# jeffreychou777/GenComm

Hardware: AMD Instinct MI355X
Metric: scenes/sec (higher is better)
Workload: dtype f32

## Files before the change

### gencomm_amd/csrc/gencomm_abi.hip

```cpp
#include "../../include/gencomm_hip.h"

#include "common.h"
#include "conv_kernels.h"
#include "detect_kernels.h"
#include "enhancer_host.h"
#include "fusion_kernels.h"
#include "msgext_host.h"
#include "noise_kernels.h"
#include "pillar_kernels.h"
#include "pfn_kernels.h"
#include "train_kernels.h"
#include "wgrad_h3_kernels.h"
#include "unet_bwd_host.h"
#include "unet_host.h"

#include <algorithm>
#include <atomic>
#include <map>
#include <mutex>
#include <string>
#include <stdlib.h>
#include <string.h>

namespace gc {
char* last_error_buf() {
  static thread_local char buf[512] = {0};
  return buf;
}
KernelTimer& kernel_timer() {
  static KernelTimer t;
  return t;
}
static std::atomic<long long> g_modes[MODE_COUNT] = {{0}, {0}, {0}, {2}, {-1}, {1}, {0}, {0}, {-1}, {1}, {16}};
static std::atomic<bool> g_klog_armed{false};
static std::mutex g_klog_mu;
static std::map<std::string, int> g_klog;
bool klog_armed() { return g_klog_armed.load(std::memory_order_relaxed); }
void klog_note(const char* name) {
  std::lock_guard<std::mutex> lk(g_klog_mu);
  ++g_klog[name];
}
Modes modes_snapshot() {
  Modes m;
  for (int i = 0; i < MODE_COUNT; ++i) m.v[i] = g_modes[i].load(std::memory_order_relaxed);
  return m;
}
}

using namespace gc;

extern "C" {

int gencomm_abi_version(void) { return GENCOMM_ABI_VERSION; }
#ifndef GENCOMM_BUILD_FLAGS
#define GENCOMM_BUILD_FLAGS "unknown"
#endif
const char* gencomm_build_info(void) { return GENCOMM_BUILD_FLAGS; }
const char* gencomm_last_error(void) { return last_error_buf(); }

int gencomm_set_mode(int key, long long value) {
  GC_CHECK_ARG(key >= 0 && key < MODE_COUNT, "unknown mode key");
  GC_CHECK_ARG(key != MODE_ARITH || (value >= 0 && value <= 3), "GENCOMM_MODE_ARITH: 0 (three-term f16-pipe path), 1 (exact fp32), 2 (bf16 denoise) or 3 (0 + two-term general convolutions)");
  GC_CHECK_ARG(key != MODE_SAMPLER || (value >= 0 && value <= 2), "GENCOMM_MODE_SAMPLER: 0 (automatic), 1 (direct) or 2 (latent)");
  GC_CHECK_ARG(key != MODE_TILE_WANT || value >= 0, "GENCOMM_MODE_TILE_WANT: 0 (automatic) or a positive workgroup count");
  GC_CHECK_ARG(key != MODE_TILE8 || value >= -1, "GENCOMM_MODE_TILE8: -1 (automatic), 0 (off) or a positive workgroup count");
  GC_CHECK_ARG(key != MODE_BWD_STREAMS || (value >= 0 && value <= 2), "GENCOMM_MODE_BWD_STREAMS: 0 (off), 1 (automatic) or 2 (always)");
  GC_CHECK_ARG(key != MODE_PERSIST || (value >= 0 && value <= 31), "GENCOMM_MODE_PERSIST: a mask of the five layer variants (0 .. 31)");
  g_modes[key].store(value, std::memory_order_relaxed);
  return GC_OK;
}
long long gencomm_get_mode(int key) {
  if (key < 0 || key >= MODE_COUNT) { fail(GC_ERR_ARG, "unknown mode key"); return -1; }
  return g_modes[key].load(std::memory_order_relaxed);
}

int gencomm_timer_num_kernels(void) { return KF_COUNT; }
const char* gencomm_timer_kernel_name(int family) { return kernel_family_name(family); }

int gencomm_timer_start_mask(unsigned long long mask, int capacity) {
  KernelTimer& t = kernel_timer();
  GC_CHECK_ARG(t.ev == nullptr, "timer already armed");
  GC_CHECK_ARG(mask != 0 && (mask >> KF_COUNT) == 0 && capacity >= 1 && capacity <= (1 << 20), "bad family mask / capacity");
  t.ev = new hipEvent_t[2 * (size_t)capacity];
  for (int i = 0; i < 2 * capacity; ++i) {
    if (hipEventCreate(&t.ev[i]) != hipSuccess) {
      for (int j = 0; j < i; ++j) (void)hipEventDestroy(t.ev[j]);
      delete[] t.ev;
      t.ev = nullptr;
      return fail(GC_ERR_HIP, "hipEventCreate failed");
    }
  }
  t.fam = new int[capacity];
  t.bytes = new double[capacity];
  t.mask = mask; t.cap = capacity; t.count = 0;
  return GC_OK;
}
int gencomm_timer_start(int family, int capacity) {
  GC_CHECK_ARG(family >= 0 && family < KF_COUNT, "bad family");
  return gencomm_timer_start_mask(1ull << family, capacity);
}

int gencomm_timer_stop_families(double* ms, int* launches, double* algorithmic_bytes, int n_families) {
  KernelTimer& t = kernel_timer();
  GC_CHECK_ARG(t.ev != nullptr, "timer not armed");
  GC_CHECK_ARG(n_families >= 0 && n_families <= KF_COUNT, "bad n_families");
  for (int f = 0; f < n_families; ++f) {
    if (ms) ms[f] = 0.0;
    if (launches) launches[f] = 0;
    if (algorithmic_bytes) algorithmic_bytes[f] = 0.0;
  }
  int rc = GC_OK;
  for (int i = 0; i < t.count; ++i) {
    float e = 0.f;
    if (hipEventSynchronize(t.ev[2 * i + 1]) != hipSuccess || hipEventElapsedTime(&e, t.ev[2 * i], t.ev[2 * i + 1]) != hipSuccess)
      rc = fail(GC_ERR_HIP, "event timing failed");
    const int f = t.fam[i];
    if (f < n_families) {
      if (ms) ms[f] += e;
      if (launches) launches[f] += 1;
      if (algorithmic_bytes) algorithmic_bytes[f] += t.bytes[i];
    }
  }
  for (int i = 0; i < 2 * t.cap; ++i) (void)hipEventDestroy(t.ev[i]);
  delete[] t.ev;
  delete[] t.fam;
  delete[] t.bytes;
  t = KernelTimer{};
  return rc;
}

int gencomm_timer_stop(double* total_ms, int* launches) {
  double ms[KF_COUNT];
  int n[KF_COUNT];
  const int rc = gencomm_timer_stop_families(ms, n, nullptr, KF_COUNT);
  double sum = 0.0;
  int cnt = 0;
  for (int f = 0; f < KF_COUNT; ++f) { sum += ms[f]; cnt += n[f]; }
  if (total_ms) *total_ms = sum;
  if (launches) *launches = cnt;
  return rc;
}

int gencomm_klog_start(void) {
  std::lock_guard<std::mutex> lk(g_klog_mu);
  g_klog.clear();
  g_klog_armed.store(true, std::memory_order_relaxed);
// ... 279 lines not shown
  prep_c16_kernel<<<cdiv(2 * 1152, 256), 256, 0, st>>>(w, scratch, transposed);
  Modes m = modes_snapshot();
  m.v[MODE_ARITH] = 1;
  const size_t plane = (size_t)H * W;
  for (int g = 0; g < 2; ++g) {
    Conv8Args a{};
    a.src[0] = x; a.src[1] = x + 8 * plane; a.src_ct = x_ct;
    a.w = scratch + g * 1152; a.bias = scratch + 2 * 1152;
    a.dst = y + (size_t)8 * g * plane; a.dst_ct = y_ct;
    a.H = a.Hin = H; a.W = a.Win = W;
    a.xcd = m.xcd();
    launch_conv8<2, false, false, 0>(m, pick_tile(m, n, H, W), a, n, st);
  }
  GC_HIP(hipGetLastError());
  return GC_OK;
}

static void launch_q_sample(const QSampleArgs& q, int n, bool philox, hipStream_t st) {
  TimedLaunch tl(KF_Q_SAMPLE, st);
  const dim3 qgrid((unsigned)std::max<long long>(1, std::min<long long>((q.per_agent / 64 + 255) / 256, 2048)), n);
  GC_KLOG(philox ? "q_sample_kernel<true> (in-kernel Philox)" : "q_sample_kernel<false> (explicit noise)");
  if (philox) q_sample_kernel<true><<<qgrid, 256, 0, st>>>(q);
  else q_sample_kernel<false><<<qgrid, 256, 0, st>>>(q);
}

int gencomm_q_sample_fwd(const float* sched_row, const float* feat, int n_feat_rows, const int* src_row,
                         const float* noise, unsigned long long seed, unsigned int stream_id,
                         float* out, int n, int C, int H, int W, void* stream) {
  GC_CHECK_ARG(sched_row && feat && src_row && out, "null pointer");
  GC_CHECK_ARG(n >= 1 && n <= 65535 && n_feat_rows >= 1 && C >= 1 && H >= 1 && W >= 1, "bad n/C/H/W");
  QSampleArgs q{feat, src_row, noise, sched_row, out, seed, stream_id, (long long)C * H * W, nullptr, nullptr};
  launch_q_sample(q, n, noise == nullptr, (hipStream_t)stream);
  GC_HIP(hipGetLastError());
  return GC_OK;
}

int gencomm_step_noise_fwd(const float* sched_row, unsigned long long seed, unsigned int stream_id, float* out,
                           int n, int C, int H, int W, int unrounded, void* stream) {
  GC_CHECK_ARG(sched_row && out, "null pointer");
  GC_CHECK_ARG(n >= 1 && n <= 65535 && C >= 2 && (C & 1) == 0 && H >= 1 && W >= 1, "bad n/C/H/W (C must be even)");
  StepNoiseArgs a{out, sched_row, seed, stream_id, C, H, W, unrounded ? 1 : 0, (long long)n * (C / 2) * H * ((W + 3) / 4)};
  const unsigned grid = (unsigned)std::max<long long>(1, std::min<long long>((a.items + 255) / 256, 65536));
  step_noise_kernel<<<grid, 256, 0, (hipStream_t)stream>>>(a);
  GC_HIP(hipGetLastError());
  return GC_OK;
}

int gencomm_denoise_fwd(const float* prepared, const float* sched,
                        const float* feat, int n_feat_rows, const int* src_row, const float* cond,
                        float* out, const float* noise0, const float* step_noise, unsigned long long seed,
                        int n, int C, int H, int W, int levels, int res_blocks, int attn_mask, int T,
                        void* workspace, long long workspace_bytes, void* stream) {
  return gencomm_denoise_fwd_dseed(prepared, sched, feat, n_feat_rows, src_row, cond, out, noise0, step_noise, seed, nullptr,
                                   n, C, H, W, levels, res_blocks, attn_mask, T, workspace, workspace_bytes, stream);
}

int gencomm_denoise_fwd_dseed(const float* prepared, const float* sched,
                              const float* feat, int n_feat_rows, const int* src_row, const float* cond,
                              float* out, const float* noise0, const float* step_noise, unsigned long long seed,
                              const unsigned long long* seed_dev,
                              int n, int C, int H, int W, int levels, int res_blocks, int attn_mask, int T,
                              void* workspace, long long workspace_bytes, void* stream) {
  UNetPlan p;
  if (const char* e = p.build(C, levels, res_blocks, attn_mask, T)) return fail(GC_ERR_ARG, e);
  if (int rc = check_dims(n, C, H, W)) return rc;
  GC_CHECK_ARG(prepared && sched && feat && src_row && cond && out && workspace, "null pointer");
  GC_CHECK_ARG(n_feat_rows >= 1, "n_feat_rows must be positive");
  GC_CHECK_ARG((noise0 == nullptr) == (step_noise == nullptr), "noise0 and step_noise must both be given or both be null");
  UNetWorkspace w;
  if (const char* e = w.build(p, n, H, W)) return fail(GC_ERR_ARG, e);
  if ((long long)w.total > workspace_bytes) return fail(GC_ERR_WORKSPACE, "workspace too small (see gencomm_denoise_workspace_bytes)");
  hipStream_t st = (hipStream_t)stream;
  const bool philox = noise0 == nullptr;
  const long long per_agent = (long long)C * H * W;

  UNetCall c{&p, &w, prepared, (char*)workspace, n, H, W, st, modes_snapshot()};
  if (int rc = check_bf16_mode(c.m, p, W)) return rc;
  GC_HIP(hipMemsetAsync(c.amax(), 0, 256, st));
  amax_kernel<<<256, 256, 0, st>>>(cond, (long long)n * 2 * H * W, c.amax());
  QSampleArgs q{feat, src_row, noise0, sched + (size_t)(T - 1) * 5, out, seed, (unsigned)T, per_agent, seed_dev, c.amax() + 1};
  launch_q_sample(q, n, philox, st);

  const long long smode = c.m.v[MODE_SAMPLER];
  const bool want_latent = smode == 2 || (smode == 0 && pick_tile(c.m, n, H, W) == TILE_64x16);
  const bool latent = want_latent && T >= 2 && (W % 4) == 0;
  if (!latent) {
    for (int i = 0; i < T; ++i) {
      const int t = T - 1 - i;
      ConvOutArgs co{};
      co.out = out;
      co.xt = out;
      co.sched = sched + (size_t)t * 5;
      co.noise = philox ? nullptr : step_noise + (size_t)i * n * per_agent;
      co.seed = seed;
      co.seed_dev = seed_dev;
      co.stream_id = (unsigned)t;
      const int post = t == 0 ? 0 : (philox ? 2 : 1);
      if (int rc = unet_enqueue(c, out, cond, t, post, co)) return rc;
    }
    return GC_OK;
  }
  const int nops = (int)p.ops.size();
  kmap_enqueue(c, cond);
  for (int i = 0; i < T; ++i) {
    const int t = T - 1 - i;
    ConvOutArgs co{};
    co.out = out;
    if (int rc = unet_enqueue_range(c, out, cond, t, 0, co, i == 0 ? 0 : 1, t == 0 ? nops : nops - 1, i != 0, i == 0)) return rc;
    if (t > 0) {
      const float* nz = philox ? nullptr : step_noise + (size_t)i * n * per_agent;
      if (int rc = latent_step_enqueue(c, sched + (size_t)t * 5, nz, seed, (unsigned)t, seed_dev)) return rc;
    }
  }
  return GC_OK;
}

int gencomm_enhancer_num_params(int C) {
  EnhancerPlan p;
  if (const char* e = p.build(C)) { fail(GC_ERR_ARG, e); return -1; }
  return (int)p.params.size();
}
int gencomm_enhancer_param_info(int C, int index, char* name, int name_cap, long long* numel, long long* offset) {
  EnhancerPlan p;
  if (const char* e = p.build(C)) return fail(GC_ERR_ARG, e);
  GC_CHECK_ARG(index >= 0 && index < (int)p.params.size(), "param index out of range");
  GC_CHECK_ARG(name && name_cap > 0 && numel && offset, "null output pointer");
  snprintf(name, (size_t)name_cap, "%s", p.params[index].name.c_str());
  *numel = p.params[index].numel;
  *offset = p.params[index].off;
  return GC_OK;
}
long long gencomm_enhancer_raw_floats(int C) {
  EnhancerPlan p;
  if (const char* e = p.build(C)) { fail(GC_ERR_ARG, e); return -1; }
  return p.raw_floats;
}
long long gencomm_enhancer_workspace_bytes(int n, int C, int H, int W) {
  EnhancerPlan p;
  if (const char* e = p.build(C)) { fail(GC_ERR_ARG, e); return -1; }
  if (n < 1 || H < 1 || W < 1) { fail(GC_ERR_ARG, "n, H, W must be positive"); return -1; }
  return (long long)enhancer_workspace_bytes(p, n, H, W);
}
int gencomm_enhancer_fwd(const float* raw, const float* x, float* out, int n, int C, int H, int W,
                         void* workspace, long long workspace_bytes, void* stream) {
  EnhancerPlan p;
  if (const char* e = p.build(C)) return fail(GC_ERR_ARG, e);
  GC_CHECK_ARG(raw && x && workspace, "null pointer");
  GC_CHECK_ARG(n >= 1 && n <= 65535 && H >= 1 && W >= 1, "bad n/H/W");
  if ((long long)enhancer_workspace_bytes(p, n, H, W) > workspace_bytes)
    return fail(GC_ERR_WORKSPACE, "workspace too small (see gencomm_enhancer_workspace_bytes)");
  return enhancer_enqueue(p, raw, x, out, n, H, W, (char*)workspace, (hipStream_t)stream, modes_snapshot());
}

int gencomm_msgext_num_params(int C) {
  MsgExtPlan p;
  if (const char* e = p.build(C)) { fail(GC_ERR_ARG, e); return -1; }
  return (int)p.params.size();
}
int gencomm_msgext_param_info(int C, int index, char* name, int name_cap, long long* numel, long long* offset) {
  MsgExtPlan p;
  if (const char* e = p.build(C)) return fail(GC_ERR_ARG, e);
  GC_CHECK_ARG(index >= 0 && index < (int)p.params.size(), "param index out of range");
  GC_CHECK_ARG(name && name_cap > 0 && numel && offset, "null output pointer");
  snprintf(name, (size_t)name_cap, "%s", p.params[index].name.c_str());
  *numel = p.params[index].numel;
  *offset = p.params[index].off;
  return GC_OK;
// ... 556 lines not shown
```

### gencomm_amd/csrc/latenth_kernels.h

```cpp
#pragma once
#include "conv8b_kernels.h"
#include "conv8h_kernels.h"
#include "latent_kernels.h"

namespace gc {

constexpr int HL_LH5 = HC_TH + 4;
constexpr int HL_PLANE5 = HL_LH5 * HC_ROW;
constexpr int HL_W5TAB3 = 8 * HC_WC3;
constexpr int HL_TPLANE5 = HL_PLANE5 / 2;
constexpr int HL_RING = (2 * (HC_TW + 4) + 2 * HL_LH5) * 8;

__global__ __launch_bounds__(256) void prep_latent_h_kernel(const float* __restrict__ wc5, const float* __restrict__ w_in ,
                                                           float* __restrict__ dst5, float* __restrict__ dstx,
                                                           float* __restrict__ dstc, int C) {
  __shared__ float s_max[256];
  const int tid = threadIdx.x;
  const int CI = C + 2;
  float m = 0.f;
  for (int i = tid; i < 1600; i += 256) m = fmaxf(m, fabsf(wc5[i]));
  for (int i = tid; i < 8 * CI * 9; i += 256) m = fmaxf(m, fabsf(w_in[i]));
  s_max[tid] = m;
  __syncthreads();
  for (int s = 128; s > 0; s >>= 1) {
// ... 337 lines not shown
    for (int i = 0; i < 4; ++i) b0[i] = (oc0 + i < C) ? a.bias[oc0 + i] * sc : 0.f;
#pragma unroll 1
    for (int rp = 0; rp < 2; ++rp) {
      f32x4 acc[2][4] = {{b0, b0, b0, b0}, {b0, b0, b0, b0}};
      const unsigned char* trow = tile + 2 * rp * HC_ROW;
#pragma unroll
      for (int c = 0; c < 3; ++c) {
        WA3 wa;
        load_wa3(wa, tab, c, lane);
        long bt[2][4];
#pragma unroll
        for (int r = 0; r < 2; ++r)
#pragma unroll
          for (int j = 0; j < 4; ++j) bt[r][j] = *reinterpret_cast<const long*>(tile + HC_TOFF + (((2 * rp + r) * HC_ROW + off[j][c]) >> 1));
#pragma unroll
        for (int r = 0; r < 2; ++r) {
          __builtin_amdgcn_sched_barrier(0);
#pragma unroll
          for (int j = 0; j < 4; ++j) acc[r][j] = __builtin_amdgcn_mfma_f32_16x16x32_bf8_bf8(wa.wb, bt[r][j], acc[r][j], 0, 0, 0);
        }
        __builtin_amdgcn_sched_barrier(0);
#pragma unroll
        for (int r = 0; r < 2; ++r) {
          half8_t bh[4], bl[4];
#pragma unroll
          for (int j = 0; j < 4; ++j) {
            bh[j] = *reinterpret_cast<const half8_t*>(trow + r * HC_ROW + off[j][c]);
            bl[j] = *reinterpret_cast<const half8_t*>(trow + r * HC_ROW + HC_PLANE + off[j][c]);
          }
#pragma unroll
          for (int j = 0; j < 4; ++j) acc[r][j] = __builtin_amdgcn_mfma_f32_16x16x32_f16(wa.w[2], bh[j], acc[r][j], 0, 0, 0);
#pragma unroll
          for (int j = 0; j < 4; ++j) acc[r][j] = __builtin_amdgcn_mfma_f32_16x16x32_f16(wa.w[1], bl[j], acc[r][j], 0, 0, 0);
#pragma unroll
          for (int j = 0; j < 4; ++j) acc[r][j] = __builtin_amdgcn_mfma_f32_16x16x32_f16(wa.w[1], bh[j], acc[r][j], 0, 0, 0);
#pragma unroll
          for (int j = 0; j < 4; ++j) acc[r][j] = __builtin_amdgcn_mfma_f32_16x16x32_f16(wa.w[0], bl[j], acc[r][j], 0, 0, 0);
#pragma unroll
          for (int j = 0; j < 4; ++j) acc[r][j] = __builtin_amdgcn_mfma_f32_16x16x32_f16(wa.w[0], bh[j], acc[r][j], 0, 0, 0);
          if (r == 0) __builtin_amdgcn_sched_barrier(0);
        }
      }
      __builtin_amdgcn_sched_barrier(0);
#pragma unroll
      for (int r = 0; r < 2; ++r) {
        const int gy = y0 + 4 * wave + 2 * rp + r;
        if (gy >= H || gx + 3 >= W) continue;
#pragma unroll
        for (int ip = 0; ip < 2; ++ip) {
          if (oc0 + 2 * ip >= C) continue;
          float z8[8];
          if (POST == 2)
            noise_pair_quad((uint64_t)(((size_t)n * C + oc0 + 2 * ip) * plane + (size_t)gy * W + gx), a.stream_id, seed, bm_k2(sg), z8);
#pragma unroll
          for (int ii = 0; ii < 2; ++ii) {
            const int i = 2 * ip + ii, oc = oc0 + i;
            const size_t e = ((size_t)n * C + oc) * plane + (size_t)gy * W + gx;
            float v[4];
#pragma unroll
            for (int j = 0; j < 4; ++j) v[j] = acc[r][j][i] * inv_s;
            if (POST != 0) {
              const float4 t4 = *reinterpret_cast<const float4*>(a.xt + e);
              const float xt[4] = {t4.x, t4.y, t4.z, t4.w};
              if (POST == 1) {
                const float4 z4 = *reinterpret_cast<const float4*>(a.noise + e);
                const float z[4] = {z4.x, z4.y, z4.z, z4.w};
#pragma unroll
                for (int j = 0; j < 4; ++j) v[j] = fmaf(sg, z[j], fmaf(c1, v[j], c2 * xt[j]));
              } else {
#pragma unroll
                for (int j = 0; j < 4; ++j) v[j] = z8[4 * ii + j] + fmaf(c1, v[j], c2 * xt[j]);
              }
            }
            *reinterpret_cast<float4*>(a.out + e) = make_float4(v[0], v[1], v[2], v[3]);
            if (POST != 0) amax = fmaxf(amax, fmaxf(fmaxf(fabsf(v[0]), fabsf(v[1])), fmaxf(fabsf(v[2]), fabsf(v[3]))));
          }
        }
      }
    }
  }
  if (POST != 0 && a.amax_out != nullptr) wave_amax_commit(amax, a.amax_out);
}

template <int NOISE>
__global__ __launch_bounds__(HC_NT, 3) void latent_step_h_kernel(const LatentArgs a) {
  constexpr int NT = HC_NT, TW = HC_TW, TH = HC_TH;
  constexpr int TILE_BYTES = NOISE == 1 ? 2 * HC_PLANE + HC_TPLANE : 2 * HL_PLANE5;
  __shared__ __align__(16) unsigned char tile[TILE_BYTES];
  __shared__ float s_ring[HL_RING];
  __shared__ float s_ab[8][2];
  __shared__ float s_red[NT / 64][16];

  fp16_ovfl_clamp();
  const int tid = threadIdx.x, lane = tid & 63, wave = tid >> 6;
  const BlockId bid = xcd_block(a.xcd);
  const int n = bid.z;
  const int x0 = bid.x * TW, y0 = bid.y * TH;
  const int H = a.H, W = a.W;
  const unsigned plane = (unsigned)(H * W);
  const float c1 = a.sched[2], c2 = a.sched[3], sg = a.sched[4];
  const unsigned long long seed = (NOISE == 2 && a.seed_dev) ? *a.seed_dev : a.seed;
  const int ln = lane & 15, g = lane >> 4, ch = g & 1, rr = g >> 1;
  const int gx = x0 + 4 * ln;
  const int gy0 = y0 + 4 * wave + rr;
  const bool wave_live = y0 + 4 * wave < H;

  const int af32 = !a.a_bf16;
  const size_t abase = (size_t)n * 8 * plane;
  float4 qm[8], qr[2];
  float hh[2][2];
  const int r0 = tid >> 4, qx = tid & 15;
  const bool ok_m = (y0 - 2 + r0) >= 0 && (y0 - 2 + r0) < H && (x0 + 4 * qx) < W;
#pragma unroll
  for (int c = 0; c < 8; ++c)
    qm[c] = ok_m ? ld4(a.a_src, af32, abase + ((unsigned)c * plane + (unsigned)(y0 - 2 + r0) * (unsigned)W + (unsigned)(x0 + 4 * qx)))
                 : make_float4(0.f, 0.f, 0.f, 0.f);
  const int rrow = TH + ((tid & 63) >> 4), cpr = tid >> 6;
  const bool ok_r = (y0 - 2 + rrow) >= 0 && (y0 - 2 + rrow) < H && (x0 + 4 * qx) < W;
#pragma unroll
  for (int k = 0; k < 2; ++k)
    qr[k] = ok_r ? ld4(a.a_src, af32, abase + ((unsigned)(2 * cpr + k) * plane + (unsigned)(y0 - 2 + rrow) * (unsigned)W + (unsigned)(x0 + 4 * qx)))
                 : make_float4(0.f, 0.f, 0.f, 0.f);
  bool ok_h[2];
#pragma unroll
  for (int j = 0; j < 2; ++j) {
    const int idx = tid + j * NT;
    const int cp = idx & 3, s = (idx >> 2) & 3, r = idx >> 4;
    const int gy = y0 - 2 + r, gxh = s < 2 ? x0 - 2 + s : x0 + TW + (s - 2);
    ok_h[j] = idx < HL_LH5 * 16 && gy >= 0 && gy < H && gxh >= 0 && gxh < W;
    hh[j][0] = hh[j][1] = 0.f;
    if (ok_h[j]) {
      hh[j][0] = ld1(a.a_src, af32, abase + (unsigned)(2 * cp) * plane + (unsigned)gy * (unsigned)W + (unsigned)gxh);
      hh[j][1] = ld1(a.a_src, af32, abase + (unsigned)(2 * cp + 1) * plane + (unsigned)gy * (unsigned)W + (unsigned)gxh);
    }
  }
  if (tid < 8) {
    float A, B;
    gn_coeff(a.a_stat + (size_t)n * 16, tid, 2, a.inv_cnt, a.gamma[tid], a.beta[tid], &A, &B);
    s_ab[tid][0] = A;
    s_ab[tid][1] = B;
  }
  __syncthreads();
  auto act = [&](int c, float v, bool ok) { return ok ? c1 * silu_f(fmaf(s_ab[c][0], v, s_ab[c][1])) : 0.f; };
  uint2 tq[4];
  uint32_t tr2[2];
  uint32_t th2;
  {
    float e[8][4];
#pragma unroll
    for (int c = 0; c < 8; ++c) {
      e[c][0] = act(c, qm[c].x, ok_m); e[c][1] = act(c, qm[c].y, ok_m); e[c][2] = act(c, qm[c].z, ok_m); e[c][3] = act(c, qm[c].w, ok_m);
    }
#pragma unroll
    for (int j = 0; j < 4; ++j) {
      uint4 hi, lo;
      float t[8];
      split3_pair(e[0][j], e[1][j], hi.x, lo.x, t[0], t[1]);
      split3_pair(e[2][j], e[3][j], hi.y, lo.y, t[2], t[3]);
      split3_pair(e[4][j], e[5][j], hi.z, lo.z, t[4], t[5]);
      split3_pair(e[6][j], e[7][j], hi.w, lo.w, t[6], t[7]);
      const int addr = r0 * HC_ROW + j * HC_PHASE + (qx + 1) * 16;
      *reinterpret_cast<uint4*>(tile + addr) = hi;
      *reinterpret_cast<uint4*>(tile + HL_PLANE5 + addr) = lo;
      tq[j] = make_uint2(bf8x4s(t[0], t[1], t[2], t[3]), bf8x4s(t[4], t[5], t[6], t[7]));
    }
  }
  {
// ... 67 lines not shown
  if (NOISE == 1) {
    stage_load<TW, TH, NT, 8, false>(R, np_, plane, W, H, W, x0, y0, tid);
    hreg = halo_load_h<false>(np_, plane, W, H, W, x0, y0, tid);
  }
  __syncthreads();

  const float inv_s = a.wc5h[HL_W5TAB3], sc = a.wc5h[HL_W5TAB3 + 1];
  f32x4 acc[2][4];
  {
    const float4 b4 = *reinterpret_cast<const float4*>(a.bsum + 4 * ch);
    const float k = c1 * sc;
    const f32x4 b0 = {b4.x * k, b4.y * k, b4.z * k, b4.w * k};
#pragma unroll
    for (int p = 0; p < 2; ++p)
#pragma unroll
      for (int j = 0; j < 4; ++j) acc[p][j] = b0;
  }
  auto addr5 = [&](int c, int p, int j) {
    const int t = min(4 * c + g, 29);
    const int dyp = t / 5, dx = t - 5 * dyp;
    const int po = j + dx - 2;
    return (4 * wave + dyp + 2 * p) * HC_ROW + (ln + 1) * 16 + (po & 3) * HC_PHASE + (po >> 2) * 16;
  };
  if (wave_live) {
#pragma unroll 2
    for (int c = 0; c < 8; ++c) {
      half8_t w[3];
#pragma unroll
      for (int k = 0; k < 3; ++k) w[k] = __builtin_bit_cast(half8_t, *reinterpret_cast<const uint4*>(a.wc5h + c * HC_WC3 + (k * 64 + lane) * 4));
#pragma unroll
      for (int p = 0; p < 2; ++p) {
        half8_t b[4];
#pragma unroll
        for (int j = 0; j < 4; ++j) b[j] = *reinterpret_cast<const half8_t*>(tile + addr5(c, p, j));
#pragma unroll
        for (int j = 0; j < 4; ++j) acc[p][j] = __builtin_amdgcn_mfma_f32_16x16x32_f16(w[2], b[j], acc[p][j], 0, 0, 0);
#pragma unroll
        for (int j = 0; j < 4; ++j) acc[p][j] = __builtin_amdgcn_mfma_f32_16x16x32_f16(w[1], b[j], acc[p][j], 0, 0, 0);
#pragma unroll
        for (int j = 0; j < 4; ++j) acc[p][j] = __builtin_amdgcn_mfma_f32_16x16x32_f16(w[0], b[j], acc[p][j], 0, 0, 0);
        __builtin_amdgcn_sched_barrier(0);
#pragma unroll
        for (int j = 0; j < 4; ++j) b[j] = *reinterpret_cast<const half8_t*>(tile + HL_PLANE5 + addr5(c, p, j));
#pragma unroll
        for (int j = 0; j < 4; ++j) acc[p][j] = __builtin_amdgcn_mfma_f32_16x16x32_f16(w[1], b[j], acc[p][j], 0, 0, 0);
#pragma unroll
        for (int j = 0; j < 4; ++j) acc[p][j] = __builtin_amdgcn_mfma_f32_16x16x32_f16(w[0], b[j], acc[p][j], 0, 0, 0);
        __builtin_amdgcn_sched_barrier(0);
      }
    }
  }

  if (wave_live) {
    hl_border_fix(a, s_ring, x0, y0, acc[0], gy0, gx, gy0 - y0, gx - x0, 4 * ch, c1, sc);
    hl_border_fix(a, s_ring, x0, y0, acc[1], gy0 + 2, gx, gy0 + 2 - y0, gx - x0, 4 * ch, c1, sc);
  }

  auto composite_third_term = [&](const unsigned char* tbase) {
    static_for<0, 8>([&](auto CC) {
      constexpr int c = decltype(CC)::value;
      const long wb = *reinterpret_cast<const long*>(a.wc5h + c * HC_WC3 + 768 + lane * 2);
      long bt[2][4];
#pragma unroll
      for (int p = 0; p < 2; ++p)
#pragma unroll
        for (int j = 0; j < 4; ++j) bt[p][j] = *reinterpret_cast<const long*>(tbase + (addr5(c, p, j) >> 1));
#pragma unroll
      for (int p = 0; p < 2; ++p) {
        __builtin_amdgcn_sched_barrier(0);
#pragma unroll
        for (int j = 0; j < 4; ++j) acc[p][j] = __builtin_amdgcn_mfma_f32_16x16x32_bf8_bf8(wb, bt[p][j], acc[p][j], 0, 0, 0);
      }
    });
    __builtin_amdgcn_sched_barrier(0);
  };
  __syncthreads();
  write_t_plane(tile + HL_PLANE5);
  __syncthreads();
  if (wave_live) composite_third_term(tile + HL_PLANE5);

  int off[4][3];
  hc_lane_offsets(off, wave, lane);
  const int nchunk = a.C / 8;
  if (NOISE == 2) {
    __syncthreads();
    write_t_plane(tile + HL_PLANE5);
  }
#pragma unroll 1
  for (int cc = 0; cc < nchunk; ++cc) {
    __syncthreads();
    const float* __restrict__ wtab = a.wxh + (size_t)cc * HC_WTAB3;
    if (NOISE == 1) {
      stage_store_h<false, true>(tile, R, hreg, H, W, x0, y0, nullptr, tid, sg);
      if (cc + 1 < nchunk) {
        stage_load<TW, TH, NT, 8, false>(R, np_ + (size_t)(cc + 1) * 8 * plane, plane, W, H, W, x0, y0, tid);
        hreg = halo_load_h<false>(np_ + (size_t)(cc + 1) * 8 * plane, plane, W, H, W, x0, y0, tid);
      }
    } else {
      const float k2 = bm_k2(sg);
      auto words = [&](int cp, int r, int gx2, NoiseWords& w) -> float {
        const int gy2 = y0 - 1 + r;
        noise_words((uint64_t)(((size_t)n * a.C + (size_t)cc * 8 + 2 * cp) * plane + (size_t)gy2 * W + gx2), a.stream_id, seed, w);
        return (gy2 >= 0 && gy2 < H && gx2 >= 0 && gx2 < W) ? k2 : 0.f;
      };
      {
        uint32_t h[4][4];
#pragma unroll
        for (int cp = 0; cp < 4; ++cp) {
          NoiseWords w;
          const float kk = words(cp, r0, x0 + 4 * qx, w);
#pragma unroll
          for (int j = 0; j < 4; ++j) h[cp][j] = bm_pair_h(w.ur[j], w.w[j], kk);
        }
#pragma unroll
        for (int j = 0; j < 4; ++j)
          *reinterpret_cast<uint4*>(tile + r0 * HC_ROW + j * HC_PHASE + (qx + 1) * 16) = make_uint4(h[0][j], h[1][j], h[2][j], h[3][j]);
      }
      {
        const int cr = tid >> 5, rrw = TH + ((tid >> 4) & 1);
        NoiseWords w;
        const float kk = words(cr >> 1, rrw, x0 + 4 * qx, w);
        const bool odd = (cr & 1) != 0;
        const int jb = odd ? 2 : 0;
        const uint32_t wsel[2] = {odd ? w.w[2] : w.w[0], odd ? w.w[3] : w.w[1]};
        const float usel[2] = {odd ? w.ur[2] : w.ur[0], odd ? w.ur[3] : w.ur[1]};
#pragma unroll
        for (int k = 0; k < 2; ++k)
          *reinterpret_cast<uint32_t*>(tile + rrw * HC_ROW + (jb + k) * HC_PHASE + (qx + 1) * 16 + (cr >> 1) * 4) = bm_pair_h(usel[k], wsel[k], kk);
      }
      if (tid < HC_LH * 8) {
        const int cp = tid & 3, side = (tid >> 2) & 1, r = tid >> 3;
        NoiseWords w;
        const float kk = words(cp, r, side ? x0 + TW : x0 - 4, w);
        *reinterpret_cast<uint32_t*>(tile + hc_addr(r, side ? HC_TW : -1) + cp * 4) = bm_pair_h(side ? w.ur[0] : w.ur[3], side ? w.w[0] : w.w[3], kk);
      }
    }
    __syncthreads();
    if (wave_live) {
      if (NOISE == 1) {
        conv_tile_mfma3(tile, wtab, acc, off, lane);
      } else {
        conv_tile_mfma3_hionly(tile, wtab, acc, off, lane);
      }
    }
  }

  float part[8];
#pragma unroll
  for (int i = 0; i < 8; ++i) part[i] = 0.f;
  if (wave_live) {
#pragma unroll
    for (int p = 0; p < 2; ++p) {
      const int gy = gy0 + 2 * p;
      if (gy < H && gx + 3 < W) {
#pragma unroll
        for (int i = 0; i < 4; ++i) {
          const size_t e = ((size_t)n * 8 + 4 * ch + i) * plane + (size_t)gy * W + gx;
          const float4 k4 = *reinterpret_cast<const float4*>(a.kmap + e);
          const float4 h4 = *reinterpret_cast<const float4*>(a.hs0 + e);
          const float kk[4] = {k4.x, k4.y, k4.z, k4.w}, hv[4] = {h4.x, h4.y, h4.z, h4.w};
          float v[4];
#pragma unroll
          for (int j = 0; j < 4; ++j) v[j] = kk[j] + c2 * (hv[j] - kk[j]) + acc[p][j][i] * inv_s;
          *reinterpret_cast<float4*>(a.hs0 + e) = make_float4(v[0], v[1], v[2], v[3]);
#pragma unroll
          for (int j = 0; j < 4; ++j) { part[i] += v[j]; part[4 + i] = fmaf(v[j], v[j], part[4 + i]); }
        }
      }
    }
  }
  hc_stats_commit(part, s_red, a.hs0_stat + (size_t)n * 16, tid);
}

}
```

### gencomm_amd/csrc/unet_host.h

```cpp
#pragma once
#include <stdlib.h>

#include "attn_kernels.h"
#include "conv8b_kernels.h"
#include "conv8h_kernels.h"
#include "conv8h8_kernels.h"
#include "dataflow_kernels.h"
#include "latent_kernels.h"
#include "latenth_kernels.h"
#include "unet_kernels.h"
#include "unet_plan.h"

namespace gc {

inline int cdiv(int a, int b) { return (a + b - 1) / b; }

enum TileCfg { TILE_64x16 = 0, TILE_32x16 = 1, TILE_32x8 = 2 };
inline long long tile_want(const Modes& m) {
  return m.v[MODE_TILE_WANT] > 0 ? m.v[MODE_TILE_WANT] : (m.split() ? 160LL : 512LL);
}
inline TileCfg pick_tile(const Modes& m, int n, int H, int W, int zmul = 1) {
  if (m.bf16()) return TILE_64x16;
  const long long want = tile_want(m);
  if ((long long)cdiv(W, 64) * cdiv(H, 16) * n * zmul >= want) return TILE_64x16;
// ... 336 lines not shown
      case OP_CONV_OUT: {
        co.src = c.tensor_ptr(o.src[0]); co.sstat = c.stat_ptr(o.src[0]);
        co.gamma = P + p.nout_w; co.beta = P + p.nout_b;
        co.w = P + p.conv_out.p_w; co.wh = P + p.conv_out.p_wh; co.bias = P + p.conv_out.b;
        co.C = p.C; co.H = Hl; co.W = Wl;
        co.inv_cnt = 1.0 / (2.0 * Hl * Wl);
        co.xcd = c.m.xcd();
        co.amax_out = post != 0 ? c.amax() + 1 : nullptr;
        co.src_bf16 = !c.is_f32(o.src[0]);
        const int nocb = (p.C + 15) / 16;
        const TileCfg tc = pick_tile(c.m, c.n, Hl, Wl, nocb) == TILE_64x16 ? TILE_64x16 : TILE_32x8;
        int tw, th;
        tile_dims(tc, &tw, &th);
        const dim3 grid(cdiv(Wl, tw), cdiv(Hl, th), c.n * nocb);
#define GC_LAUNCH_CO(POST)                                                             \
  do {                                                                                 \
    if (tc == TILE_64x16) conv_out_kernel<64, 16, 4, POST><<<grid, 256, 0, c.st>>>(co); \
    else conv_out_kernel<32, 8, 1, POST><<<grid, 256, 0, c.st>>>(co);                  \
  } while (0)
        TimedLaunch tl(KF_CONV_OUT, c.st);
        if (c.m.split() && (Wl & 3) == 0 && pick_tile(c.m, c.n, Hl, Wl) == TILE_64x16) {
          const dim3 gh(cdiv(Wl, 64), cdiv(Hl, 16), c.n);
          GC_KLOG(post == 0 ? "conv_out_h_kernel<0> (x0_hat)" : post == 1 ? "conv_out_h_kernel<1> (explicit noise)" : "conv_out_h_kernel<2> (in-kernel Philox)");
          if (post == 0) conv_out_h_kernel<0><<<gh, 256, 0, c.st>>>(co);
          else if (post == 1) conv_out_h_kernel<1><<<gh, 256, 0, c.st>>>(co);
          else conv_out_h_kernel<2><<<gh, 256, 0, c.st>>>(co);
        } else {
          GC_KLOG(post == 0 ? "conv_out_kernel<tile,0> (exact fp32, x0_hat)" : post == 1 ? "conv_out_kernel<tile,1> (exact fp32, explicit noise)" : "conv_out_kernel<tile,2> (exact fp32, in-kernel Philox)");
          if (post == 0) GC_LAUNCH_CO(0);
          else if (post == 1) GC_LAUNCH_CO(1);
          else GC_LAUNCH_CO(2);
        }
#undef GC_LAUNCH_CO
        break;
      }
    }
  }
  GC_HIP(hipGetLastError());
  return GC_OK;
}

inline int unet_enqueue(const UNetCall& c, const float* x_t, const float* cond, int t, int post, ConvOutArgs co) {
  return unet_enqueue_range(c, x_t, cond, t, post, co, 0, (int)c.plan->ops.size(), false);
}

inline void kmap_enqueue(const UNetCall& c, const float* cond) {
  const UNetPlan& p = *c.plan;
  ConvInArgs a{cond, nullptr, c.prepared + p.conv_in.p_w, c.prepared + p.conv_in.b,
               reinterpret_cast<float*>(c.wsp + c.ws->kmap_off), nullptr, 0, c.H, c.W, c.m.xcd()};
  const TileCfg tc = pick_tile(c.m, c.n, c.H, c.W);
  int tw, th;
  tile_dims(tc, &tw, &th);
  const dim3 grid(cdiv(c.W, tw), cdiv(c.H, th), c.n);
  if (tc == TILE_64x16 && c.m.split() && (c.W & 3) == 0) {
    ConvInHArgs ah{cond, nullptr, c.prepared + p.p_wch, c.prepared + p.p_wxh, c.prepared + p.p_wc5h + HL_W5TAB3, c.prepared + p.conv_in.b,
                   reinterpret_cast<float*>(c.wsp + c.ws->kmap_off), nullptr, 0, c.H, c.W, c.m.xcd(), c.amax()};
    conv_in_h_kernel<<<grid, 256, 0, c.st>>>(ah);
  } else if (tc == TILE_64x16) conv_in_kernel<64, 16, 4><<<grid, 256, 0, c.st>>>(a);
  else if (tc == TILE_32x16) conv_in_kernel<32, 16, 4><<<grid, 128, 0, c.st>>>(a);
  else conv_in_kernel<32, 8, 1><<<grid, 256, 0, c.st>>>(a);
}

inline int latent_step_enqueue(const UNetCall& c, const float* sched_row, const float* noise, unsigned long long seed,
                               unsigned stream_id, const unsigned long long* seed_dev = nullptr) {
  const UNetPlan& p = *c.plan;
  const float* P = c.prepared;
  GC_HIP(hipMemsetAsync(c.stat_ptr(p.hs0_tensor), 0, (size_t)c.n * 16 * sizeof(double), c.st));
  LatentArgs a{};
  a.a_src = c.tensor_ptr(p.last_body_tensor); a.a_stat = c.stat_ptr(p.last_body_tensor);
  a.gamma = P + p.nout_w; a.beta = P + p.nout_b;
  a.kmap = reinterpret_cast<const float*>(c.wsp + c.ws->kmap_off);
  a.hs0 = c.tensor_ptr(p.hs0_tensor); a.hs0_stat = c.stat_ptr(p.hs0_tensor);
  a.wc5 = P + p.p_wc5; a.wc1 = P + p.p_wc1; a.bring = P + p.p_bring; a.bsum = P + p.p_bsum;
  a.wx = P + p.conv_in.p_w + 144;
  a.wc5h = P + p.p_wc5h; a.wxh = P + p.p_wxh;
  a.noise = noise; a.sched = sched_row; a.inv_cnt = 1.0 / (2.0 * c.H * c.W);
  a.seed = seed; a.seed_dev = seed_dev; a.stream_id = stream_id; a.C = p.C; a.H = c.H; a.W = c.W;
  a.xcd = c.m.xcd();
  a.a_bf16 = !c.is_f32(p.last_body_tensor);
  TimedLaunch tl(KF_LATENT_STEP, c.st, 4.0 * c.n * 32.0 * c.H * c.W);
  const bool small_h = c.m.split() && (c.W & 3) == 0 && c.W >= 64 && c.H >= 16 && c.m.v[MODE_TILE_WANT] == 0;
  if ((pick_tile(c.m, c.n, c.H, c.W) == TILE_64x16 || small_h) && c.m.split()) {
    const dim3 grid(cdiv(c.W, 64), cdiv(c.H, 16), c.n);
    GC_KLOG(noise ? "latent_step_h_kernel<1> (explicit noise)" : "latent_step_h_kernel<2> (in-kernel Philox)");
    if (noise) latent_step_h_kernel<1><<<grid, 256, 0, c.st>>>(a);
    else latent_step_h_kernel<2><<<grid, 256, 0, c.st>>>(a);
  } else if (pick_tile(c.m, c.n, c.H, c.W) == TILE_64x16) {
    const dim3 grid(cdiv(c.W, 64), cdiv(c.H, 16), c.n);
    GC_KLOG(noise ? "latent_step_kernel<64,16,1> (exact fp32, explicit noise)" : "latent_step_kernel<64,16,2> (exact fp32, in-kernel Philox)");
    if (noise) latent_step_kernel<64, 16, 1><<<grid, 256, 0, c.st>>>(a);
    else latent_step_kernel<64, 16, 2><<<grid, 256, 0, c.st>>>(a);
  } else {
    const dim3 grid(cdiv(c.W, 32), cdiv(c.H, 16), c.n);
    GC_KLOG(noise ? "latent_step_kernel<32,16,1> (exact fp32, explicit noise)" : "latent_step_kernel<32,16,2> (exact fp32, in-kernel Philox)");
    if (noise) latent_step_kernel<32, 16, 1><<<grid, 128, 0, c.st>>>(a);
    else latent_step_kernel<32, 16, 2><<<grid, 128, 0, c.st>>>(a);
  }
  GC_HIP(hipGetLastError());
  return GC_OK;
}

inline int unet_prepare_enqueue(const UNetPlan& p, const float* raw, float* prepared, hipStream_t st) {
  GC_HIP(hipMemcpyAsync(prepared, raw, (size_t)p.raw_floats * sizeof(float), hipMemcpyDeviceToDevice, st));
  auto conv_w = [&](long long src, long long dst, int OC, int IC, int OCB) {
    const int total = OC * IC * 9;
    prep_conv_w_kernel<<<cdiv(total, 256), 256, 0, st>>>(raw + src, prepared + dst, OC, IC, OCB);
  };
  conv_w(p.conv_in.w, p.conv_in.p_w, 8, p.C + 2, 8);
  GC_HIP(hipMemsetAsync(prepared + p.conv_out.p_w, 0, (size_t)((p.C + 15) / 16 * 16) * 72 * sizeof(float), st));
  conv_w(p.conv_out.w, p.conv_out.p_w, p.C, 8, 16);
  prep_conv_out_h_kernel<<<1, 256, 0, st>>>(raw + p.conv_out.w, prepared + p.conv_out.p_wh, p.C);
  for (int l = 0; l < p.L; ++l) {
    if (p.down[l].w >= 0) conv_w(p.down[l].w, p.down[l].p_w, 8, 8, 8);
    if (p.up[l].w >= 0) {
      conv_w(p.up[l].w, p.up[l].p_w, 8, 8, 8);
      prep_conv8h_kernel<<<1, 256, 0, st>>>(raw + p.up[l].w, prepared + p.up[l].p_wh, 8);
      prep_conv8b_kernel<<<1, 256, 0, st>>>(raw + p.up[l].w, prepared + p.up[l].p_wb, 8);
    }
  }
  TembArgs ta{};
  ta.raw = raw; ta.prepared = prepared;
  ta.d0w = p.d0w; ta.d0b = p.d0b; ta.d1w = p.d1w; ta.d1b = p.d1b;
  ta.nblocks = (int)p.blocks.size(); ta.T = p.T;
  for (size_t i = 0; i < p.blocks.size(); ++i) {
    const ResBlockPlan& b = p.blocks[i];
    conv_w(b.c1w, b.p_c1w, 8, b.cin, 8);
    conv_w(b.c2w, b.p_c2w, 8, 8, 8);
    prep_conv8h_kernel<<<1, 256, 0, st>>>(raw + b.c1w, prepared + b.p_c1wh, b.cin);
    prep_conv8h_kernel<<<1, 256, 0, st>>>(raw + b.c2w, prepared + b.p_c2wh, 8);
    prep_conv8b_kernel<<<1, 256, 0, st>>>(raw + b.c1w, prepared + b.p_c1wb, b.cin);
    prep_conv8b_kernel<<<1, 256, 0, st>>>(raw + b.c2w, prepared + b.p_c2wb, 8);
    if (b.cin != 8) prep_nin_w_kernel<<<1, 256, 0, st>>>(raw + b.ninw, prepared + b.p_ninw, 8, b.cin);
    prep_add_kernel<<<1, 64, 0, st>>>(raw + b.c2b, b.cin != 8 ? raw + b.ninb : nullptr, prepared + b.p_bias2, 8);
    ta.tpw[i] = b.tpw; ta.tpb[i] = b.tpb; ta.c1b[i] = b.c1b; ta.dst[i] = b.p_bias1;
  }
  prep_temb_kernel<<<p.T, 64, 0, st>>>(ta);
  {
    PrepLatentArgs la{raw + p.conv_in.w, raw + p.conv_out.w, raw + p.conv_out.b, prepared + p.p_wc5, prepared + p.p_wc1,
                      prepared + p.p_bring, prepared + p.p_bsum, p.C};
    prep_latent_kernel<<<cdiv(1600 + 5184 + 72 + 8, 256), 256, 0, st>>>(la);
    prep_latent_h_kernel<<<1, 256, 0, st>>>(prepared + p.p_wc5, raw + p.conv_in.w, prepared + p.p_wc5h, prepared + p.p_wxh,
                                           prepared + p.p_wch, p.C);
  }
  GC_HIP(hipGetLastError());
  return GC_OK;
}

}
```

Before: 188.7.

## Double-buffer in-kernel Philox noise planes in latent step to drop a barrier

```diff
diff --git a/gencomm_amd/csrc/gencomm_abi.hip b/gencomm_amd/csrc/gencomm_abi.hip
--- a/gencomm_amd/csrc/gencomm_abi.hip
+++ b/gencomm_amd/csrc/gencomm_abi.hip
@@ -61,7 +61,7 @@
 int gencomm_set_mode(int key, long long value) {
   GC_CHECK_ARG(key >= 0 && key < MODE_COUNT, "unknown mode key");
   GC_CHECK_ARG(key != MODE_ARITH || (value >= 0 && value <= 3), "GENCOMM_MODE_ARITH: 0 (three-term f16-pipe path), 1 (exact fp32), 2 (bf16 denoise) or 3 (0 + two-term general convolutions)");
-  GC_CHECK_ARG(key != MODE_SAMPLER || (value >= 0 && value <= 2), "GENCOMM_MODE_SAMPLER: 0 (automatic), 1 (direct) or 2 (latent)");
+  GC_CHECK_ARG(key != MODE_SAMPLER || (value >= 0 && value <= 3), "GENCOMM_MODE_SAMPLER: 0 (automatic), 1 (direct), 2 (latent) or 3 (latent, retained step body)");
   GC_CHECK_ARG(key != MODE_TILE_WANT || value >= 0, "GENCOMM_MODE_TILE_WANT: 0 (automatic) or a positive workgroup count");
   GC_CHECK_ARG(key != MODE_TILE8 || value >= -1, "GENCOMM_MODE_TILE8: -1 (automatic), 0 (off) or a positive workgroup count");
   GC_CHECK_ARG(key != MODE_BWD_STREAMS || (value >= 0 && value <= 2), "GENCOMM_MODE_BWD_STREAMS: 0 (off), 1 (automatic) or 2 (always)");
@@ -507,7 +507,7 @@
   launch_q_sample(q, n, philox, st);
 
   const long long smode = c.m.v[MODE_SAMPLER];
-  const bool want_latent = smode == 2 || (smode == 0 && pick_tile(c.m, n, H, W) == TILE_64x16);
+  const bool want_latent = smode >= 2 || (smode == 0 && pick_tile(c.m, n, H, W) == TILE_64x16);
   const bool latent = want_latent && T >= 2 && (W % 4) == 0;
   if (!latent) {
     for (int i = 0; i < T; ++i) {
diff --git a/gencomm_amd/csrc/latenth_kernels.h b/gencomm_amd/csrc/latenth_kernels.h
--- a/gencomm_amd/csrc/latenth_kernels.h
+++ b/gencomm_amd/csrc/latenth_kernels.h
@@ -443,7 +443,7 @@
   if (POST != 0 && a.amax_out != nullptr) wave_amax_commit(amax, a.amax_out);
 }
 
-template <int NOISE>
+template <int NOISE, bool OLD = false>
 __global__ __launch_bounds__(HC_NT, 3) void latent_step_h_kernel(const LatentArgs a) {
   constexpr int NT = HC_NT, TW = HC_TW, TH = HC_TH;
   constexpr int TILE_BYTES = NOISE == 1 ? 2 * HC_PLANE + HC_TPLANE : 2 * HL_PLANE5;
@@ -677,65 +677,78 @@
   int off[4][3];
   hc_lane_offsets(off, wave, lane);
   const int nchunk = a.C / 8;
-  if (NOISE == 2) {
-    __syncthreads();
-    write_t_plane(tile + HL_PLANE5);
-  }
+  auto gen_noise = [&](unsigned char* buf, int cc) {
+    const float k2 = bm_k2(sg);
+    auto words = [&](int cp, int r, int gx2, NoiseWords& w) -> float {
+      const int gy2 = y0 - 1 + r;
+      noise_words((uint64_t)(((size_t)n * a.C + (size_t)cc * 8 + 2 * cp) * plane + (size_t)gy2 * W + gx2), a.stream_id, seed, w);
+      return (gy2 >= 0 && gy2 < H && gx2 >= 0 && gx2 < W) ? k2 : 0.f;
+    };
+    {
+      uint32_t h[4][4];
+#pragma unroll
+      for (int cp = 0; cp < 4; ++cp) {
+        NoiseWords w;
+        const float kk = words(cp, r0, x0 + 4 * qx, w);
+#pragma unroll
+        for (int j = 0; j < 4; ++j) h[cp][j] = bm_pair_h(w.ur[j], w.w[j], kk);
+      }
+#pragma unroll
+      for (int j = 0; j < 4; ++j)
+        *reinterpret_cast<uint4*>(buf + r0 * HC_ROW + j * HC_PHASE + (qx + 1) * 16) = make_uint4(h[0][j], h[1][j], h[2][j], h[3][j]);
+    }
+    {
+      const int cr = tid >> 5, rrw = TH + ((tid >> 4) & 1);
+      NoiseWords w;
+      const float kk = words(cr >> 1, rrw, x0 + 4 * qx, w);
+      const bool odd = (cr & 1) != 0;
+      const int jb = odd ? 2 : 0;
+      const uint32_t wsel[2] = {odd ? w.w[2] : w.w[0], odd ? w.w[3] : w.w[1]};
+      const float usel[2] = {odd ? w.ur[2] : w.ur[0], odd ? w.ur[3] : w.ur[1]};
+#pragma unroll
+      for (int k = 0; k < 2; ++k)
+        *reinterpret_cast<uint32_t*>(buf + rrw * HC_ROW + (jb + k) * HC_PHASE + (qx + 1) * 16 + (cr >> 1) * 4) = bm_pair_h(usel[k], wsel[k], kk);
+    }
+    if (tid < HC_LH * 8) {
+      const int cp = tid & 3, side = (tid >> 2) & 1, r = tid >> 3;
+      NoiseWords w;
+      const float kk = words(cp, r, side ? x0 + TW : x0 - 4, w);
+      *reinterpret_cast<uint32_t*>(buf + hc_addr(r, side ? HC_TW : -1) + cp * 4) = bm_pair_h(side ? w.ur[0] : w.ur[3], side ? w.w[0] : w.w[3], kk);
+    }
+  };
+  if constexpr (NOISE == 2 && !OLD) {
+    if (nchunk > 0) gen_noise(tile, 0);
 #pragma unroll 1
-  for (int cc = 0; cc < nchunk; ++cc) {
-    __syncthreads();
-    const float* __restrict__ wtab = a.wxh + (size_t)cc * HC_WTAB3;
-    if (NOISE == 1) {
-      stage_store_h<false, true>(tile, R, hreg, H, W, x0, y0, nullptr, tid, sg);
-      if (cc + 1 < nchunk) {
-        stage_load<TW, TH, NT, 8, false>(R, np_ + (size_t)(cc + 1) * 8 * plane, plane, W, H, W, x0, y0, tid);
-        hreg = halo_load_h<false>(np_ + (size_t)(cc + 1) * 8 * plane, plane, W, H, W, x0, y0, tid);
-      }
-    } else {
-      const float k2 = bm_k2(sg);
-      auto words = [&](int cp, int r, int gx2, NoiseWords& w) -> float {
-        const int gy2 = y0 - 1 + r;
-        noise_words((uint64_t)(((size_t)n * a.C + (size_t)cc * 8 + 2 * cp) * plane + (size_t)gy2 * W + gx2), a.stream_id, seed, w);
-        return (gy2 >= 0 && gy2 < H && gx2 >= 0 && gx2 < W) ? k2 : 0.f;
-      };
-      {
-        uint32_t h[4][4];
-#pragma unroll
-        for (int cp = 0; cp < 4; ++cp) {
-          NoiseWords w;
-          const float kk = words(cp, r0, x0 + 4 * qx, w);
-#pragma unroll
-          for (int j = 0; j < 4; ++j) h[cp][j] = bm_pair_h(w.ur[j], w.w[j], kk);
-        }
-#pragma unroll
-        for (int j = 0; j < 4; ++j)
-          *reinterpret_cast<uint4*>(tile + r0 * HC_ROW + j * HC_PHASE + (qx + 1) * 16) = make_uint4(h[0][j], h[1][j], h[2][j], h[3][j]);
-      }
-      {
-        const int cr = tid >> 5, rrw = TH + ((tid >> 4) & 1);
-        NoiseWords w;
-        const float kk = words(cr >> 1, rrw, x0 + 4 * qx, w);
-        const bool odd = (cr & 1) != 0;
-        const int jb = odd ? 2 : 0;
-        const uint32_t wsel[2] = {odd ? w.w[2] : w.w[0], odd ? w.w[3] : w.w[1]};
-        const float usel[2] = {odd ? w.ur[2] : w.ur[0], odd ? w.ur[3] : w.ur[1]};
-#pragma unroll
-        for (int k = 0; k < 2; ++k)
-          *reinterpret_cast<uint32_t*>(tile + rrw * HC_ROW + (jb + k) * HC_PHASE + (qx + 1) * 16 + (cr >> 1) * 4) = bm_pair_h(usel[k], wsel[k], kk);
-      }
-      if (tid < HC_LH * 8) {
-        const int cp = tid & 3, side = (tid >> 2) & 1, r = tid >> 3;
-        NoiseWords w;
-        const float kk = words(cp, r, side ? x0 + TW : x0 - 4, w);
-        *reinterpret_cast<uint32_t*>(tile + hc_addr(r, side ? HC_TW : -1) + cp * 4) = bm_pair_h(side ? w.ur[0] : w.ur[3], side ? w.w[0] : w.w[3], kk);
-      }
-    }
-    __syncthreads();
-    if (wave_live) {
+    for (int cc = 0; cc < nchunk; ++cc) {
+      __syncthreads();
+      if (wave_live) conv_tile_mfma3_hionly(tile + (cc & 1) * HL_PLANE5, a.wxh + (size_t)cc * HC_WTAB3, acc, off, lane);
+      if (cc + 1 < nchunk) gen_noise(tile + ((cc + 1) & 1) * HL_PLANE5, cc + 1);
+    }
+  } else {
+    if (NOISE == 2) {
+      __syncthreads();
+      write_t_plane(tile + HL_PLANE5);
+    }
+#pragma unroll 1
+    for (int cc = 0; cc < nchunk; ++cc) {
+      __syncthreads();
+      const float* __restrict__ wtab = a.wxh + (size_t)cc * HC_WTAB3;
       if (NOISE == 1) {
-        conv_tile_mfma3(tile, wtab, acc, off, lane);
+        stage_store_h<false, true>(tile, R, hreg, H, W, x0, y0, nullptr, tid, sg);
+        if (cc + 1 < nchunk) {
+          stage_load<TW, TH, NT, 8, false>(R, np_ + (size_t)(cc + 1) * 8 * plane, plane, W, H, W, x0, y0, tid);
+          hreg = halo_load_h<false>(np_ + (size_t)(cc + 1) * 8 * plane, plane, W, H, W, x0, y0, tid);
+        }
       } else {
-        conv_tile_mfma3_hionly(tile, wtab, acc, off, lane);
+        gen_noise(tile, cc);
+      }
+      __syncthreads();
+      if (wave_live) {
+        if (NOISE == 1) {
+          conv_tile_mfma3(tile, wtab, acc, off, lane);
+        } else {
+          conv_tile_mfma3_hionly(tile, wtab, acc, off, lane);
+        }
       }
     }
   }
diff --git a/gencomm_amd/csrc/unet_host.h b/gencomm_amd/csrc/unet_host.h
--- a/gencomm_amd/csrc/unet_host.h
+++ b/gencomm_amd/csrc/unet_host.h
@@ -442,8 +442,11 @@
   const bool small_h = c.m.split() && (c.W & 3) == 0 && c.W >= 64 && c.H >= 16 && c.m.v[MODE_TILE_WANT] == 0;
   if ((pick_tile(c.m, c.n, c.H, c.W) == TILE_64x16 || small_h) && c.m.split()) {
     const dim3 grid(cdiv(c.W, 64), cdiv(c.H, 16), c.n);
-    GC_KLOG(noise ? "latent_step_h_kernel<1> (explicit noise)" : "latent_step_h_kernel<2> (in-kernel Philox)");
+    const bool old_body = !noise && c.m.v[MODE_SAMPLER] == 3;
+    GC_KLOG(noise ? "latent_step_h_kernel<1> (explicit noise)"
+                  : old_body ? "latent_step_h_kernel<2, old> (in-kernel Philox, two-barrier chunk loop)" : "latent_step_h_kernel<2> (in-kernel Philox)");
     if (noise) latent_step_h_kernel<1><<<grid, 256, 0, c.st>>>(a);
+    else if (old_body) latent_step_h_kernel<2, true><<<grid, 256, 0, c.st>>>(a);
     else latent_step_h_kernel<2><<<grid, 256, 0, c.st>>>(a);
   } else if (pick_tile(c.m, c.n, c.H, c.W) == TILE_64x16) {
     const dim3 grid(cdiv(c.W, 64), cdiv(c.H, 16), c.n);
```

Result: no change. 189.9 (median of 2 runs) (+0.7%).
